# hzxie/RMNet

Measured on AMD Instinct MI355X. Metric: frames/sec at 480p, 1 object, T=5 memory; memory-read HBM GB/s vs peak, higher is better.
Workload: dtype f32 convs; memory read = fp16 operands (K, V, q, P rounded to 11 bits), fp32 accumulate (RMNET_BANK_F16): the frame loop's default for clips with one object -- on one-object 480x854 clips whose masks HAVE a boundary (tests/live_fixture.py) mask IoU vs the CPU path 0.99993-0.99997 and foreground logi

## Files before the change

### include/rmnet_hip.h

```cpp
#ifndef RMNET_HIP_H_
#define RMNET_HIP_H_

#include <stddef.h>
#include <stdint.h>

#ifdef __cplusplus
extern "C" {
#endif

#define RMNET_ABI_VERSION 6

enum {
  RMNET_OK = 0,
  RMNET_E_INVALID_ARG = -1,
  RMNET_E_WORKSPACE = -2,
  RMNET_E_LAUNCH = -3,
  RMNET_E_UNSUPPORTED = -4
};

int rmnet_abi_version(void);
const char *rmnet_error_string(int code);

size_t rmnet_region_map_workspace_bytes(int B, int K, int H, int W);
int rmnet_region_map_f32(const float *mask, int B, int K, int H, int W, float prob_threshold,
                         int n_pts_threshold, int n_bbox_loose_pixels, float *att_map,
                         int32_t *bboxes, int32_t *cell_rects, int pad_l, int pad_t,
                         int cell_stride, int cells_h, int cells_w, void *workspace,
                         size_t workspace_bytes, void *stream);

int rmnet_region_map_warped_f32(const float *mask, const float *flow, int B, int K, int H, int W,
                                float prob_threshold, int n_pts_threshold, int n_bbox_loose_pixels,
                                float *att_map, int32_t *bboxes, int32_t *cell_rects, int pad_l,
                                int pad_t, int cell_stride, int cells_h, int cells_w, float *warped,
                                void *workspace, size_t workspace_bytes, void *stream);

int rmnet_boxes_to_cell_rects_i32(const int32_t *bboxes, int n_boxes, int k_per_batch, int pad_l,
                                  int pad_t, int cell_stride, int cells_h, int cells_w,
                                  int32_t *cell_rects, void *stream);

#define RMNET_MR_DEFAULT 0
#define RMNET_MR_FORCE_GENERIC 1
#define RMNET_MR_EXACT_FP32 2
#define RMNET_MR_F16 4
#define RMNET_BANK_F16 4
#define RMNET_MR_QX 8
#define RMNET_BANK_QX 8

size_t rmnet_memory_read_workspace_bytes(int no, int De, int Do, int T, int h, int w, int flags);
int rmnet_memory_read_f32(const float *m_key, const float *m_val, const float *q_key,
                          const float *q_val, int no, int De, int Do, int T, int h, int w,
                          long long m_chan_stride, long long m_obj_stride, long long v_chan_stride,
                          long long v_obj_stride, float *mem_val, float *p_out,
                          const int32_t *mem_rects, const int32_t *qry_rects, int flags,
                          void *workspace, size_t workspace_bytes, void *stream);

int rmnet_memory_read_f32_ev(const float *m_key, const float *m_val, const float *q_key,
                             const float *q_val, int no, int De, int Do, int T, int h, int w,
                             long long m_chan_stride, long long m_obj_stride,
                             long long v_chan_stride, long long v_obj_stride, float *mem_val,
                             float *p_out, const int32_t *mem_rects, const int32_t *qry_rects,
                             int flags, void *workspace, size_t workspace_bytes, void *stream,
                             void *ev_start, void *ev_mid, void *ev_end);

size_t rmnet_bank_bytes(int no, int Tcap, int h, int w);
size_t rmnet_bank_overflow_offset(int no, int Tcap, int h, int w);
size_t rmnet_bank_area_offset(int no, int Tcap, int h, int w);
int rmnet_bank_append_f32(void *bank, int no, int Tcap, int h, int w, int slot, const float *k4,
                          const float *v4, const int32_t *rects, void *stream);
int rmnet_bank_append_f32_at(void *bank, int no, int Tcap, int h, int w, int slot, const int32_t *slot_dev,
                             const float *k4, const float *v4, const int32_t *rects, void *stream);
int rmnet_bank_read_f32_at(void *bank, int no, int Tcap, int h, int w, int T, const int32_t *T_dev, int flags,
                           const float *q_key, const float *q_val, const int32_t *qry_rects,
                           float *mem_val, void *workspace, size_t workspace_bytes, void *stream,
                           void *ev_start, void *ev_mid, void *ev_end);
size_t rmnet_bank_read_workspace_bytes(int no, int h, int w);
size_t rmnet_bank_read_workspace_bytes_for(int no, int h, int w, int T);
int rmnet_bank_read_f32(void *bank, int no, int Tcap, int h, int w, int T,
                        const float *q_key, const float *q_val, const int32_t *qry_rects,
                        float *mem_val, void *workspace, size_t workspace_bytes, void *stream,
                        void *ev_start, void *ev_mid, void *ev_end);

int rmnet_rect_mask_f32(const float *x, int n, int C, int T, int h, int w, const int32_t *rects,
                        float *y, void *stream);

int rmnet_channel_affine_f32(const float *x, const float *scale, const float *shift,
                             const float *res, const float *res_scale, const float *res_shift,
                             int relu, long long N, int C, long long HW, float *out, void *stream);

int rmnet_affine_relu_maxpool_f32(const float *x, const float *scale, const float *shift, long long N,
                                  int C, int H, int W, float *out, void *stream);

int rmnet_upsample2x_add_f32(const float *x, const float *skip, long long N, int C, int h, int w,
                             float *out, void *stream);

int rmnet_channel_affine_nhwc_f32(const float *x, const float *scale, const float *shift, const float *res, const float *res_scale,
                                  const float *res_shift, int relu, long long rows, int C, float *out, void *stream);
int rmnet_upsample2x_add_nhwc_f32(const float *x, const float *skip, long long N, int C, int h, int w, float *out, void *stream);
int rmnet_affine_relu_maxpool_nhwc_f32(const float *x, const float *scale, const float *shift, long long N, int C, int H, int W,
                                       float *out, void *stream);

#define RMNET_CONV_RELU_IN 1
#define RMNET_CONV_RELU_OUT 2
int rmnet_conv3x3_split_f32(const float *x, const void *wpack, const float *w_unscale, const float *bias, const float *res, int flags,
                            int N, int H, int W, int Cin, float *out, int32_t *range_word, void *stream);

int rmnet_conv3x3_split_lds_f32(const float *x, const void *wpack, const float *w_unscale, const float *bias, const float *res,
                                int flags, int N, int H, int W, int Cin, float *out, int32_t *range_word, void *stream);

int rmnet_conv3x3_rows_f32(const float *x, const void *wpack, const float *w_unscale, const float *bias, const float *res, int flags,
                           int N, int H, int W, int Cin, float *out, int32_t *range_word, void *stream);

int rmnet_conv_split_f32(const float *x, const void *wpack, const float *w_unscale, const float *shift, const float *res, int flags,
                         int N, int H, int W, int Cin, int Cout, int ksize, int stride, float *out, float *out2, int out_split,
                         int32_t *range_word, void *stream);

#define RMNET_CONV_X_SPLIT 4
#define RMNET_CONV_OUT_SPLIT 8
int rmnet_conv_split_pre_f32(const void *x, const void *wpack, const float *w_unscale, const float *shift, const float *res, int flags,
                             int N, int H, int W, int Cin, int Cout, int ksize, int stride, void *out, float *out2, int out_split,
                             int32_t *range_word, void *stream);
int rmnet_split_act_f32(const float *x, long long M, int C, int relu, void *out, int32_t *range_word, void *stream);

int rmnet_stem_split_f32(const float *frame, const float *mask, const float *other, const void *wpack, const float *w_unscale,
                         const float *shift, int N, int H, int W, float *out, int32_t *range_word, void *stream);

int rmnet_pred_head_f32(const float *x, const float *w, const float *bias, int n, int Hq, int Wq, int C, float *out, void *stream);

#define RMNET_FLOW_RELU 1
#define RMNET_FLOW_LEAKY 2
#define RMNET_FLOW_TRANSPOSED 4
int rmnet_flow_conv_f32(const float *x, int x_ld, const void *wpack, const float *w_unscale, const float *shift, int flags, int N, int H,
                        int W, int Cin, int Cout, int ksize, int stride, float *out, int out_ld, int coff, int32_t *range_word,
                        void *stream);

size_t rmnet_flow_head_workspace_bytes(int N, int H, int W, int Cin);
int rmnet_flow_head_f32(const float *x, int x_ld, const float *wpack, const float *bias, int N, int H, int W, int Cin, float *out,
                        void *workspace, size_t workspace_bytes, void *stream);

int rmnet_flow_up_f32(const float *flow, const float *w, int N, int h, int w_, float *out, int out_ld, int coff, void *stream);

int rmnet_soft_aggregate_f32(const float *dec, const int32_t *obj_begin, int B, int K, int Hp, int Wp,
                             int pad_l, int pad_t, int H, int W, float *logit, float *prob,
                             void *stream);

int rmnet_flow_affine_f32(const float *flow, const float *m1, const float *m2, int H, int W,
                          float *out, void *stream);
size_t rmnet_flow_affine_workspace_bytes(int H, int W);
int rmnet_flow_affine_f32_host(const float *flow_host, const float *m1_host, const float *m2_host,
                               int H, int W, float *out_host, void *workspace,
                               size_t workspace_bytes, void *stream);

#ifdef __cplusplus
}
#endif
#endif
```

### rmnet_amd/_lib.py

```python

import ctypes
import os

_HERE = os.path.dirname(os.path.abspath(__file__))
LIB_PATH = os.environ.get('RMNET_HIP_LIB') or os.path.join(_HERE, 'librmnet_hip.so')

c_f32p = ctypes.c_void_p
c_i32p = ctypes.c_void_p

SIGNATURES = {
    'rmnet_abi_version': (ctypes.c_int, []),
    'rmnet_error_string': (ctypes.c_char_p, [ctypes.c_int]),
    'rmnet_region_map_workspace_bytes': (ctypes.c_size_t, [ctypes.c_int] * 4),
    'rmnet_region_map_f32': (ctypes.c_int, [
        c_f32p, ctypes.c_int, ctypes.c_int, ctypes.c_int, ctypes.c_int, ctypes.c_float, ctypes.c_int,
        ctypes.c_int, c_f32p, c_i32p, c_i32p, ctypes.c_int, ctypes.c_int, ctypes.c_int, ctypes.c_int,
        ctypes.c_int, ctypes.c_void_p, ctypes.c_size_t, ctypes.c_void_p]),
    'rmnet_region_map_warped_f32': (ctypes.c_int, [
        c_f32p, c_f32p, ctypes.c_int, ctypes.c_int, ctypes.c_int, ctypes.c_int, ctypes.c_float, ctypes.c_int,
        ctypes.c_int, c_f32p, c_i32p, c_i32p, ctypes.c_int, ctypes.c_int, ctypes.c_int, ctypes.c_int,
        ctypes.c_int, c_f32p, ctypes.c_void_p, ctypes.c_size_t, ctypes.c_void_p]),
    'rmnet_boxes_to_cell_rects_i32': (ctypes.c_int, [
        c_i32p, ctypes.c_int, ctypes.c_int, ctypes.c_int, ctypes.c_int, ctypes.c_int, ctypes.c_int,
        ctypes.c_int, c_i32p, ctypes.c_void_p]),
    'rmnet_memory_read_workspace_bytes': (ctypes.c_size_t, [ctypes.c_int] * 7),
    'rmnet_memory_read_f32': (ctypes.c_int, [
        c_f32p, c_f32p, c_f32p, c_f32p, ctypes.c_int, ctypes.c_int, ctypes.c_int, ctypes.c_int,
        ctypes.c_int, ctypes.c_int, ctypes.c_longlong, ctypes.c_longlong, ctypes.c_longlong,
        ctypes.c_longlong, c_f32p, c_f32p, c_i32p, c_i32p, ctypes.c_int, ctypes.c_void_p,
        ctypes.c_size_t, ctypes.c_void_p]),
    'rmnet_memory_read_f32_ev': (ctypes.c_int, [
        c_f32p, c_f32p, c_f32p, c_f32p, ctypes.c_int, ctypes.c_int, ctypes.c_int, ctypes.c_int,
        ctypes.c_int, ctypes.c_int, ctypes.c_longlong, ctypes.c_longlong, ctypes.c_longlong,
        ctypes.c_longlong, c_f32p, c_f32p, c_i32p, c_i32p, ctypes.c_int, ctypes.c_void_p,
        ctypes.c_size_t, ctypes.c_void_p, ctypes.c_void_p, ctypes.c_void_p, ctypes.c_void_p]),
    'rmnet_bank_bytes': (ctypes.c_size_t, [ctypes.c_int] * 4),
    'rmnet_bank_overflow_offset': (ctypes.c_size_t, [ctypes.c_int] * 4),
    'rmnet_bank_area_offset': (ctypes.c_size_t, [ctypes.c_int] * 4),
    'rmnet_bank_append_f32': (ctypes.c_int, [
        ctypes.c_void_p, ctypes.c_int, ctypes.c_int, ctypes.c_int, ctypes.c_int, ctypes.c_int, c_f32p,
        c_f32p, c_i32p, ctypes.c_void_p]),
    'rmnet_bank_append_f32_at': (ctypes.c_int, [
        ctypes.c_void_p, ctypes.c_int, ctypes.c_int, ctypes.c_int, ctypes.c_int, ctypes.c_int, c_i32p, c_f32p,
        c_f32p, c_i32p, ctypes.c_void_p]),
    'rmnet_bank_read_f32_at': (ctypes.c_int, [
        ctypes.c_void_p, ctypes.c_int, ctypes.c_int, ctypes.c_int, ctypes.c_int, ctypes.c_int, c_i32p, ctypes.c_int, c_f32p,
        c_f32p, c_i32p, c_f32p, ctypes.c_void_p, ctypes.c_size_t, ctypes.c_void_p, ctypes.c_void_p,
        ctypes.c_void_p, ctypes.c_void_p]),
    'rmnet_bank_read_workspace_bytes': (ctypes.c_size_t, [ctypes.c_int] * 3),
    'rmnet_bank_read_workspace_bytes_for': (ctypes.c_size_t, [ctypes.c_int] * 4),
    'rmnet_bank_read_f32': (ctypes.c_int, [
        ctypes.c_void_p, ctypes.c_int, ctypes.c_int, ctypes.c_int, ctypes.c_int, ctypes.c_int, c_f32p,
        c_f32p, c_i32p, c_f32p, ctypes.c_void_p, ctypes.c_size_t, ctypes.c_void_p, ctypes.c_void_p,
        ctypes.c_void_p, ctypes.c_void_p]),
    'rmnet_rect_mask_f32': (ctypes.c_int, [
        c_f32p, ctypes.c_int, ctypes.c_int, ctypes.c_int, ctypes.c_int, ctypes.c_int, c_i32p, c_f32p,
        ctypes.c_void_p]),
    'rmnet_channel_affine_f32': (ctypes.c_int, [
        c_f32p, c_f32p, c_f32p, c_f32p, c_f32p, c_f32p, ctypes.c_int, ctypes.c_longlong, ctypes.c_int,
        ctypes.c_longlong, c_f32p, ctypes.c_void_p]),
    'rmnet_upsample2x_add_f32': (ctypes.c_int, [
        c_f32p, c_f32p, ctypes.c_longlong, ctypes.c_int, ctypes.c_int, ctypes.c_int, c_f32p, ctypes.c_void_p]),
    'rmnet_soft_aggregate_f32': (ctypes.c_int, [
        c_f32p, c_i32p, ctypes.c_int, ctypes.c_int, ctypes.c_int, ctypes.c_int, ctypes.c_int, ctypes.c_int,
        ctypes.c_int, ctypes.c_int, c_f32p, c_f32p, ctypes.c_void_p]),
    'rmnet_affine_relu_maxpool_f32': (ctypes.c_int, [
        c_f32p, c_f32p, c_f32p, ctypes.c_longlong, ctypes.c_int, ctypes.c_int, ctypes.c_int, c_f32p,
        ctypes.c_void_p]),
    'rmnet_channel_affine_nhwc_f32': (ctypes.c_int, [
        c_f32p, c_f32p, c_f32p, c_f32p, c_f32p, c_f32p, ctypes.c_int, ctypes.c_longlong, ctypes.c_int, c_f32p, ctypes.c_void_p]),
    'rmnet_upsample2x_add_nhwc_f32': (ctypes.c_int, [
        c_f32p, c_f32p, ctypes.c_longlong, ctypes.c_int, ctypes.c_int, ctypes.c_int, c_f32p, ctypes.c_void_p]),
    'rmnet_affine_relu_maxpool_nhwc_f32': (ctypes.c_int, [
        c_f32p, c_f32p, c_f32p, ctypes.c_longlong, ctypes.c_int, ctypes.c_int, ctypes.c_int, c_f32p, ctypes.c_void_p]),
    'rmnet_conv3x3_split_f32': (ctypes.c_int, [
        c_f32p, ctypes.c_void_p, c_f32p, c_f32p, c_f32p, ctypes.c_int, ctypes.c_int, ctypes.c_int, ctypes.c_int, ctypes.c_int,
        c_f32p, c_i32p, ctypes.c_void_p]),
    'rmnet_conv3x3_split_lds_f32': (ctypes.c_int, [
        c_f32p, ctypes.c_void_p, c_f32p, c_f32p, c_f32p, ctypes.c_int, ctypes.c_int, ctypes.c_int, ctypes.c_int, ctypes.c_int,
        c_f32p, c_i32p, ctypes.c_void_p]),
    'rmnet_conv3x3_rows_f32': (ctypes.c_int, [
        c_f32p, ctypes.c_void_p, c_f32p, c_f32p, c_f32p, ctypes.c_int, ctypes.c_int, ctypes.c_int, ctypes.c_int, ctypes.c_int,
        c_f32p, c_i32p, ctypes.c_void_p]),
    'rmnet_conv_split_f32': (ctypes.c_int, [
        c_f32p, ctypes.c_void_p, c_f32p, c_f32p, c_f32p, ctypes.c_int, ctypes.c_int, ctypes.c_int, ctypes.c_int, ctypes.c_int,
        ctypes.c_int, ctypes.c_int, ctypes.c_int, c_f32p, c_f32p, ctypes.c_int, c_i32p, ctypes.c_void_p]),
    'rmnet_conv_split_pre_f32': (ctypes.c_int, [
        ctypes.c_void_p, ctypes.c_void_p, c_f32p, c_f32p, c_f32p, ctypes.c_int, ctypes.c_int, ctypes.c_int, ctypes.c_int, ctypes.c_int,
        ctypes.c_int, ctypes.c_int, ctypes.c_int, ctypes.c_void_p, c_f32p, ctypes.c_int, c_i32p, ctypes.c_void_p]),
    'rmnet_split_act_f32': (ctypes.c_int, [
        c_f32p, ctypes.c_longlong, ctypes.c_int, ctypes.c_int, ctypes.c_void_p, c_i32p, ctypes.c_void_p]),
    'rmnet_stem_split_f32': (ctypes.c_int, [
        c_f32p, c_f32p, c_f32p, ctypes.c_void_p, c_f32p, c_f32p, ctypes.c_int, ctypes.c_int, ctypes.c_int, c_f32p, c_i32p,
        ctypes.c_void_p]),
    'rmnet_pred_head_f32': (ctypes.c_int, [
        c_f32p, c_f32p, c_f32p, ctypes.c_int, ctypes.c_int, ctypes.c_int, ctypes.c_int, c_f32p, ctypes.c_void_p]),
    'rmnet_flow_conv_f32': (ctypes.c_int, [
        c_f32p, ctypes.c_int, ctypes.c_void_p, c_f32p, c_f32p, ctypes.c_int, ctypes.c_int, ctypes.c_int, ctypes.c_int, ctypes.c_int,
        ctypes.c_int, ctypes.c_int, ctypes.c_int, c_f32p, ctypes.c_int, ctypes.c_int, c_i32p, ctypes.c_void_p]),
    'rmnet_flow_head_workspace_bytes': (ctypes.c_size_t, [ctypes.c_int] * 4),
    'rmnet_flow_head_f32': (ctypes.c_int, [
        c_f32p, ctypes.c_int, c_f32p, c_f32p, ctypes.c_int, ctypes.c_int, ctypes.c_int, ctypes.c_int, c_f32p, ctypes.c_void_p,
        ctypes.c_size_t, ctypes.c_void_p]),
    'rmnet_flow_up_f32': (ctypes.c_int, [
        c_f32p, c_f32p, ctypes.c_int, ctypes.c_int, ctypes.c_int, c_f32p, ctypes.c_int, ctypes.c_int, ctypes.c_void_p]),
    'rmnet_flow_affine_f32': (ctypes.c_int, [
        c_f32p, c_f32p, c_f32p, ctypes.c_int, ctypes.c_int, c_f32p, ctypes.c_void_p]),
    'rmnet_flow_affine_workspace_bytes': (ctypes.c_size_t, [ctypes.c_int, ctypes.c_int]),
    'rmnet_flow_affine_f32_host': (ctypes.c_int, [
        ctypes.c_void_p, ctypes.c_void_p, ctypes.c_void_p, ctypes.c_int, ctypes.c_int,
        ctypes.c_void_p, ctypes.c_void_p, ctypes.c_size_t, ctypes.c_void_p]),
}

ABI_VERSION = 6
_lib = None


class RMNetHipError(RuntimeError):
    pass


def load():
    global _lib
    if _lib is not None:
        return _lib
    if not os.path.exists(LIB_PATH):
        raise RMNetHipError(
            'librmnet_hip.so is missing (%s). The HIP kernels are the only implementation of this '
            'path; build them with `python -m rmnet_amd.build`.' % LIB_PATH)
    lib = ctypes.CDLL(LIB_PATH)
    for name, (res, args) in SIGNATURES.items():
        fn = getattr(lib, name)
        fn.restype = res
        fn.argtypes = args
    if lib.rmnet_abi_version() != ABI_VERSION:
        raise RMNetHipError('librmnet_hip.so ABI %d != expected %d' % (lib.rmnet_abi_version(), ABI_VERSION))
    _lib = lib
    return lib


def check(code, what):
    if code != 0:
        msg = load().rmnet_error_string(code).decode()
        raise RMNetHipError('%s failed: %s (code %d)' % (what, msg, code))
```

### rmnet_amd/build.py

```python

import os
import shutil
import subprocess

HERE = os.path.dirname(os.path.abspath(__file__))
CSRC = os.path.join(HERE, 'csrc')
SOURCES = ['capi.hip', 'region_map.hip', 'flow_affine.hip', 'memory_read.hip', 'bank.hip', 'epilogue.hip', 'conv3x3.hip', 'conv3x3_rows.hip', 'conv_split.hip',
           'stem.hip', 'pred_head.hip', 'flow_conv.hip', 'flow_head.hip']
LIB = os.path.join(HERE, 'librmnet_hip.so')
ARCH = 'gfx950'


def hipcc_path():
    for cand in (shutil.which('hipcc'), '/opt/rocm/bin/hipcc'):
        if cand and os.path.exists(cand):
            return cand
    raise RuntimeError('hipcc not found: librmnet_hip.so cannot be built')


def needs_build():
    if not os.path.exists(LIB):
        return True
    t = os.path.getmtime(LIB)
    deps = [os.path.join(CSRC, s) for s in SOURCES] + [
        os.path.join(CSRC, 'common.h'),
        os.path.join(os.path.dirname(HERE), 'include', 'rmnet_hip.h')]
    return any(os.path.getmtime(d) > t for d in deps)


def build_library(force=False, verbose=False):
    if not force and not needs_build():
        return LIB
    cmd = [hipcc_path(), '--offload-arch=' + ARCH, '-O3', '-std=c++17', '-shared', '-fPIC',
           '-o', LIB] + [os.path.join(CSRC, s) for s in SOURCES]
    if verbose:
        print(' '.join(cmd))
    subprocess.check_call(cmd, cwd=CSRC)
    return LIB


if __name__ == '__main__':
    print(build_library(force=True, verbose=True))
```

### rmnet_amd/ops.py

```python

import ctypes
import os

import numpy as np
import torch

from . import _lib


MR_FORCE_GENERIC = 1
MR_EXACT_FP32 = 2
BANK_MAX_SLOTS = 2048


def _check(t, name, dtype=torch.float32):
    if not isinstance(t, torch.Tensor):
        raise RuntimeError('%s must be a torch.Tensor' % name)
    if not t.is_cuda:
        raise RuntimeError('%s must be a CUDA tensor' % name)
    if not t.is_contiguous():
        raise RuntimeError('%s must be contiguous' % name)
    if t.dtype != dtype:
        raise RuntimeError('%s must be %s, got %s' % (name, dtype, t.dtype))

# ... 447 lines not shown
    amax = w.abs().amax(dim=(1, 2, 3))
    _, ex = torch.frexp(amax)
    e = torch.where(amax > 0, 15 - ex, torch.zeros_like(ex))
    ws = torch.ldexp(w, e.view(-1, 1, 1, 1).to(w.dtype))
    hi = ws.half()
    lo = (ws - hi.float()).half()
    planes = torch.stack([p.reshape(CONV_COUT, cin // 32, 32, 9).permute(3, 1, 0, 2) for p in (hi, lo)], dim=2)
    unscale = torch.ldexp(torch.ones_like(amax), (-e).to(amax.dtype))
    return planes.contiguous().view(-1).view(torch.int16), unscale.contiguous()


_range_words = {}


def conv_range_word(device):
    idx = torch.device(device).index
    idx = torch.cuda.current_device() if idx is None else idx
    w = _range_words.get(idx)
    if w is None:
        w = _range_words[idx] = torch.zeros(1, dtype=torch.int32, device=torch.device('cuda', idx))
    return w


CONV3X3_KERNEL_DEFAULT = 'wreg'
CONV3X3_ENTRIES = {'wreg': 'rmnet_conv3x3_split_f32', 'lds': 'rmnet_conv3x3_split_lds_f32'}


def conv3x3_entry():
    v = os.environ.get('RMNET_CONV3X3_KERNEL')
    v = CONV3X3_KERNEL_DEFAULT if v is None else v.strip()
    if v not in CONV3X3_ENTRIES:
        raise RuntimeError('RMNET_CONV3X3_KERNEL must be one of %s, got %r' % (sorted(CONV3X3_ENTRIES), v))
    return CONV3X3_ENTRIES[v]


CONV3X3_ROWS_DEFAULT = True
CONV3X3_ROWS_ENTRY = 'rmnet_conv3x3_rows_f32'
CONV3X3_ROWS_CIN = 256


def conv3x3_rows_enabled():
    v = os.environ.get('RMNET_CONV3X3_ROWS')
    if v is None:
        return CONV3X3_ROWS_DEFAULT
    if v.strip() not in ('0', '1'):
        raise RuntimeError("RMNET_CONV3X3_ROWS must be '0' or '1', got %r" % v)
    return v.strip() == '1'


def conv3x3_split(x, wpack, w_unscale, bias=None, res=None, relu_in=False, relu_out=False, out=None, range_word=None):
    _check_act(x, 'x')
    if x.dim() != 4 or not x.is_contiguous(memory_format=torch.channels_last):
        raise RuntimeError('x must be a channels-last [N, Cin, H, W] tensor')
    N, cin, H, W = x.shape
    if cin % 32:
        raise RuntimeError('conv3x3_split needs Cin % 32 == 0, got %d' % cin)
    _check(wpack, 'wpack', torch.int16)
    if wpack.numel() != 9 * cin * CONV_COUT * 2:
        raise RuntimeError('wpack has %d elements, a Cin = %d pack has %d' % (wpack.numel(), cin, 9 * cin * CONV_COUT * 2))
    _check(w_unscale, 'w_unscale')
    shape = (N, CONV_COUT, H, W)
    for t, n in ((bias, 'bias'),):
        if t is not None:
            _check(t, n)
            if t.numel() != CONV_COUT:
                raise RuntimeError('%s must have 256 elements' % n)
    if w_unscale.numel() != CONV_COUT:
        raise RuntimeError('w_unscale must have 256 elements')
    if res is not None:
        _check_act(res, 'res')
        if tuple(res.shape) != shape or not res.is_contiguous(memory_format=torch.channels_last):
            raise RuntimeError('res must be a channels-last [N, 256, H, W] tensor')
    if out is None:
        out = torch.empty(shape, dtype=x.dtype, device=x.device, memory_format=torch.channels_last)
    else:
        _check_act(out, 'out')
        if tuple(out.shape) != shape or not out.is_contiguous(memory_format=torch.channels_last):
            raise RuntimeError('out must be a channels-last [N, 256, H, W] tensor')
    if range_word is not None:
        _check(range_word, 'range_word', torch.int32)
    for t in (wpack, w_unscale, bias, res, out, range_word):
        if t is not None and t.device != x.device:
            raise RuntimeError('conv3x3_split: every tensor must be on %s' % x.device)
    flags = (CONV_RELU_IN if relu_in else 0) | (CONV_RELU_OUT if relu_out else 0)
    entry = conv3x3_entry()
    if conv3x3_rows_enabled() and os.environ.get('RMNET_CONV3X3_KERNEL') is None and cin == CONV3X3_ROWS_CIN:
        entry = CONV3X3_ROWS_ENTRY
    lib = _lib.load()
    with torch.cuda.device(x.device):
        rc = getattr(lib, entry)(_ptr(x), _ptr(wpack), _ptr(w_unscale), _ptr(bias), _ptr(res), flags, N, H, W, cin,
                                 _ptr(out), _ptr(range_word), _stream(x.device))
    _lib.check(rc, entry)
    return out


@torch.no_grad()
def conv_split_pack(weight, bn_scale=None):
    if weight.dim() != 4 or weight.shape[2] != weight.shape[3] or weight.shape[2] not in (1, 3) or weight.shape[1] % 32 \
            or weight.shape[0] % 64:
        raise RuntimeError('conv_split_pack needs a [Cout, Cin, k, k] weight with k in (1, 3), Cin % 32 == 0 and Cout % 64 == 0, '
                           'got %s' % (tuple(weight.shape),))
    if weight.dtype != torch.float32:
        raise RuntimeError('conv_split_pack needs fp32 weights, got %s' % weight.dtype)
    cout, cin, k = weight.shape[0], weight.shape[1], weight.shape[2]
    w = weight.detach().double()
    if bn_scale is not None:
        if bn_scale.numel() != cout:
            raise RuntimeError('bn_scale must have Cout = %d elements' % cout)
        w = w * bn_scale.detach().to(w.device, torch.float64).view(-1, 1, 1, 1)
    amax = w.abs().amax(dim=(1, 2, 3))
    _, ex = torch.frexp(amax)
    e = torch.where(amax > 0, 15 - ex, torch.zeros_like(ex))
    ws = torch.ldexp(w, e.view(-1, 1, 1, 1).to(w.dtype))
    hi = ws.half()
    lo = (ws - hi.double()).half()
    planes = torch.stack([p.reshape(cout, cin // 32, 32, k * k).permute(3, 1, 0, 2) for p in (hi, lo)], dim=2)
    unscale = torch.ldexp(torch.ones_like(amax), (-e).to(amax.dtype)).float()
    return planes.contiguous().view(-1).view(torch.int16), unscale.contiguous()


CONV_X_SPLIT, CONV_OUT_SPLIT = 4, 8


def is_split_act(t):
    return isinstance(t, torch.Tensor) and t.dtype == torch.float16 and t.dim() == 6 and tuple(t.shape[4:]) == (2, 32)


def _check_split_act(t, name):
    if not is_split_act(t):
        raise RuntimeError('%s must be a split activation: torch.float16 [N, H, W, C // 32, 2, 32]' % name)
    if not t.is_cuda:
        raise RuntimeError('%s must be a CUDA tensor' % name)
    if not t.is_contiguous():
        raise RuntimeError('%s must be contiguous' % name)


def split_act(x, relu=False, range_word=None):
    _check_act(x, 'x')
    if x.dim() != 4 or not x.is_contiguous(memory_format=torch.channels_last):
        raise RuntimeError('x must be a channels-last [N, C, H, W] tensor')
    N, C, H, W = x.shape
    if C % 32 or x.numel() == 0:
        raise RuntimeError('split_act needs C % 32 == 0 and a non-empty tensor, got %s' % (tuple(x.shape),))
    if range_word is not None:
        _check(range_word, 'range_word', torch.int32)
        if range_word.device != x.device:
            raise RuntimeError('split_act: every tensor must be on %s' % x.device)
    out = torch.empty((N, H, W, C // 32, 2, 32), dtype=torch.float16, device=x.device)
    lib = _lib.load()
    with torch.cuda.device(x.device):
        rc = lib.rmnet_split_act_f32(_ptr(x), N * H * W, C, 1 if relu else 0, _ptr(out), _ptr(range_word), _stream(x.device))
    _lib.check(rc, 'rmnet_split_act_f32')
    return out


def conv_split(x, wpack, w_unscale, shift=None, res=None, ksize=3, stride=1, relu_in=False, relu_out=False, out=None,
               range_word=None, split=None, out_presplit=False):
    x_split = is_split_act(x)
    if x_split:
        _check_split_act(x, 'x')
        N, H, W = x.shape[:3]
        cin = x.shape[3] * 32
        if relu_in:
            raise RuntimeError('conv_split: relu_in cannot be applied to a split activation (its producer applies it)')
    else:
        _check_act(x, 'x')
        if x.dim() != 4 or not x.is_contiguous(memory_format=torch.channels_last):
            raise RuntimeError('x must be a channels-last [N, Cin, H, W] tensor')
        N, cin, H, W = x.shape
    if ksize not in (1, 3) or stride not in (1, 2):
        raise RuntimeError('conv_split implements ksize 1 / 3 and stride 1 / 2, got %r / %r' % (ksize, stride))
    _check(w_unscale, 'w_unscale')
    cout = w_unscale.numel()
    if cin % 32 or cout % 64 or cout == 0:
        raise RuntimeError('conv_split needs Cin % 32 == 0 and Cout % 64 == 0, got %d, %d' % (cin, cout))
    _check(wpack, 'wpack', torch.int16)
    if wpack.numel() != ksize * ksize * cin * cout * 2:
        raise RuntimeError('wpack has %d elements, a %dx%d Cin = %d Cout = %d pack has %d'
                           % (wpack.numel(), ksize, ksize, cin, cout, ksize * ksize * cin * cout * 2))
    pad = ksize // 2
    shape = (N, cout, (H + 2 * pad - ksize) // stride + 1, (W + 2 * pad - ksize) // stride + 1)
    if shift is not None:
        _check(shift, 'shift')
        if shift.numel() != cout:
            raise RuntimeError('shift must have Cout = %d elements' % cout)
    if res is not None:
        _check_act(res, 'res')
        if tuple(res.shape) != shape or not res.is_contiguous(memory_format=torch.channels_last):
            raise RuntimeError('res must be a channels-last %s tensor' % (shape,))
    out2 = None
    if out_presplit:
        if split is not None or out is not None:
            raise RuntimeError('conv_split: out_presplit returns one new split activation, without split / out')
        out = torch.empty((N, shape[2], shape[3], cout // 32, 2, 32), dtype=torch.float16, device=x.device)
    elif split is not None:
        if res is not None or out is not None or not 0 < split < cout or split % 4:
            raise RuntimeError('conv_split: split must be a multiple of 4 in (0, %d), without res / out' % cout)
        out = torch.empty((N, split) + shape[2:], dtype=torch.float32, device=x.device, memory_format=torch.channels_last)
        out2 = torch.empty((N, cout - split) + shape[2:], dtype=torch.float32, device=x.device, memory_format=torch.channels_last)
    elif out is None:
        out = torch.empty(shape, dtype=torch.float32, device=x.device, memory_format=torch.channels_last)
    else:
        _check_act(out, 'out')
        if tuple(out.shape) != shape or not out.is_contiguous(memory_format=torch.channels_last):
            raise RuntimeError('out must be a channels-last %s tensor' % (shape,))
    if range_word is not None:
        _check(range_word, 'range_word', torch.int32)
    for t in (wpack, w_unscale, shift, res, out, range_word):
        if t is not None and t.device != x.device:
            raise RuntimeError('conv_split: every tensor must be on %s' % x.device)
    flags = (CONV_RELU_IN if relu_in else 0) | (CONV_RELU_OUT if relu_out else 0)
    lib = _lib.load()
    with torch.cuda.device(x.device):
        if x_split or out_presplit:
            flags |= (CONV_X_SPLIT if x_split else 0) | (CONV_OUT_SPLIT if out_presplit else 0)
            what = 'rmnet_conv_split_pre_f32'
            rc = lib.rmnet_conv_split_pre_f32(_ptr(x), _ptr(wpack), _ptr(w_unscale), _ptr(shift), _ptr(res), flags, N, H, W, cin,
                                              cout, ksize, stride, _ptr(out), _ptr(out2), split or 0, _ptr(range_word),
                                              _stream(x.device))
        else:
            what = 'rmnet_conv_split_f32'
            rc = lib.rmnet_conv_split_f32(_ptr(x), _ptr(wpack), _ptr(w_unscale), _ptr(shift), _ptr(res), flags, N, H, W, cin, cout,
                                          ksize, stride, _ptr(out), _ptr(out2), split or 0, _ptr(range_word), _stream(x.device))
    _lib.check(rc, what)
    return out if out2 is None else (out, out2)


FLOW_RELU, FLOW_LEAKY, FLOW_TRANSPOSED = 1, 2, 4
_FLOW_ACT = {None: 0, False: 0, 'none': 0, True: FLOW_RELU, 'relu': FLOW_RELU, 'leaky': FLOW_LEAKY}


def flow_conv_phase_weights(weight):
    w = weight.permute(1, 0, 2, 3)
    phases = []
    for a in (0, 1):
        for b in (0, 1):
            ky = torch.tensor([3 - a, 1 - a], device=w.device)
            kx = torch.tensor([3 - b, 1 - b], device=w.device)
            phases.append(w.index_select(2, ky).index_select(3, kx))
    return torch.stack(phases, 0)


@torch.no_grad()
def flow_conv_pack(weight, transposed=False):
    if weight.dim() != 4 or weight.shape[2] != weight.shape[3] or weight.shape[2] not in ((4,) if transposed else (3, 5)):
        raise RuntimeError('flow_conv_pack needs a [Cout, Cin, k, k] weight with k in (3, 5), or transposed a [Cin, Cout, 4, 4] one, '
                           'got %s' % (tuple(weight.shape),))
    if weight.dtype != torch.float32:
        raise RuntimeError('flow_conv_pack needs fp32 weights, got %s' % weight.dtype)
    w = weight.detach().double()
    w = flow_conv_phase_weights(w) if transposed else w.unsqueeze(0)
    P, cout, cin, kh, kw = w.shape
    if cout % 64:
        raise RuntimeError('flow_conv_pack needs Cout % 64 == 0, got ' + str(cout))
    cp = (cin + 31) // 32 * 32
    amax = w.abs().amax(dim=(0, 2, 3, 4))
    _, ex = torch.frexp(amax)
    e = torch.where(amax > 0, 15 - ex, torch.zeros_like(ex))
    ws = torch.ldexp(w, e.view(1, -1, 1, 1, 1).to(w.dtype))
    hi = ws.half()
    lo = (ws - hi.double()).half()
    pad = lambda p: torch.nn.functional.pad(p, (0, 0, 0, 0, 0, cp - cin))
    planes = torch.stack([pad(p).reshape(P, cout, cp // 32, 32, kh * kw).permute(0, 4, 2, 1, 3) for p in (hi, lo)], dim=3)
    unscale = torch.ldexp(torch.ones_like(amax), (-e).to(amax.dtype)).float()
    return planes.contiguous().view(-1).view(torch.int16), unscale.contiguous()


def flow_conv_out_hw(H, W, ksize, stride, transposed):
    if transposed:
        return 2 * H, 2 * W
    pad = ksize // 2
    return (H + 2 * pad - ksize) // stride + 1, (W + 2 * pad - ksize) // stride + 1


def flow_conv(x, wpack, w_unscale, shift=None, *, ksize=3, stride=1, transposed=False, act=None, cin=None, out=None, out_coff=0,
              range_word=None):
    _check_act(x, 'x')
    if x.dim() != 4 or not x.is_contiguous(memory_format=torch.channels_last):
        raise RuntimeError('x must be a channels-last [N, C, H, W] tensor')
    if transposed:
        if ksize != 4 or stride != 2:
            raise RuntimeError('flow_conv implements the transposed convolution for ksize 4 / stride 2, got %r / %r' % (ksize, stride))
    elif ksize not in (3, 5) or stride not in (1, 2):
        raise RuntimeError('flow_conv implements ksize 3 / 5 and stride 1 / 2, got %r / %r' % (ksize, stride))
    if act not in _FLOW_ACT:
        raise RuntimeError("act must be None, 'relu' or 'leaky', got %r" % (act,))
    N, x_ld, H, W = x.shape
    cin = x_ld if cin is None else int(cin)
    cp = (cin + 31) // 32 * 32
    if cin <= 0 or x_ld % 4 or x_ld < cp:
        raise RuntimeError('flow_conv needs x_ld %% 4 == 0 and x_ld >= ceil32(cin): x has %d channels for cin = %d' % (x_ld, cin))
    _check(w_unscale, 'w_unscale')
    cout = w_unscale.numel()
    if cout % 64 or cout == 0:
        raise RuntimeError('flow_conv needs Cout % 64 == 0, got ' + str(cout))
    _check(wpack, 'wpack', torch.int16)
    want = (16 if transposed else ksize * ksize) * cp * cout * 2
    if wpack.numel() != want:
        raise RuntimeError('wpack has %d elements, a %dx%d%s cin = %d Cout = %d pack has %d'
                           % (wpack.numel(), ksize, ksize, ' transposed' if transposed else '', cin, cout, want))
    if shift is not None:
        _check(shift, 'shift')
        if shift.numel() != cout:
            raise RuntimeError('shift must have Cout = %d elements' % cout)
    Ho, Wo = flow_conv_out_hw(H, W, ksize, stride, transposed)
    if out is None:
        if out_coff:
            raise RuntimeError('out_coff without out')
        out = torch.empty((N, cout, Ho, Wo), dtype=x.dtype, device=x.device, memory_format=torch.channels_last)
    else:
        _check_act(out, 'out')
        if out.dim() != 4 or not out.is_contiguous(memory_format=torch.channels_last) or \
                (out.shape[0], out.shape[2], out.shape[3]) != (N, Ho, Wo):
            raise RuntimeError('out must be a channels-last [%d, out_ld, %d, %d] tensor' % (N, Ho, Wo))
        if out.shape[1] % 4 or out_coff % 4 or out_coff < 0 or out_coff + cout > out.shape[1]:
            raise RuntimeError('flow_conv needs out_ld %% 4 == 0, out_coff %% 4 == 0 and out_coff + Cout <= out_ld, got %d, %d, %d'
                               % (out.shape[1], out_coff, cout))
    if range_word is not None:
        _check(range_word, 'range_word', torch.int32)
    for t in (wpack, w_unscale, shift, out, range_word):
        if t is not None and t.device != x.device:
            raise RuntimeError('flow_conv: every tensor must be on %s' % x.device)
    flags = _FLOW_ACT[act] | (FLOW_TRANSPOSED if transposed else 0)
    lib = _lib.load()
    with torch.cuda.device(x.device):
        rc = lib.rmnet_flow_conv_f32(_ptr(x), x_ld, _ptr(wpack), _ptr(w_unscale), _ptr(shift), flags, N, H, W, cin, cout, ksize, stride,
                                     _ptr(out), out.shape[1], out_coff, _ptr(range_word), _stream(x.device))
    _lib.check(rc, 'rmnet_flow_conv_f32')
    return out


FLOW_HEAD_SLICE = 32


@torch.no_grad()
def flow_head_pack(weight):
    if not isinstance(weight, torch.Tensor) or weight.dim() != 4 or weight.shape[0] != 2 or tuple(weight.shape[2:]) != (3, 3) \
            or weight.shape[1] < 1:
        raise RuntimeError('flow_head_pack needs a [2, Cin, 3, 3] weight, got %s' % (tuple(getattr(weight, 'shape', ())),))
    if weight.dtype != torch.float32:
        raise RuntimeError('flow_head_pack needs fp32 weights, got %s' % weight.dtype)
    cin = weight.shape[1]
    cp = (cin + FLOW_HEAD_SLICE - 1) // FLOW_HEAD_SLICE * FLOW_HEAD_SLICE
    pack = torch.zeros(cp, 9, 2, dtype=torch.float32, device=weight.device)
    pack[:cin] = weight.detach().permute(1, 2, 3, 0).reshape(cin, 9, 2)
    return pack.view(-1)


def flow_head(x, wpack, bias, cin=None):
    _check_act(x, 'x')
    if x.dim() != 4 or not x.is_contiguous(memory_format=torch.channels_last):
        raise RuntimeError('x must be a channels-last [N, C, H, W] tensor')
    N, x_ld, H, W = x.shape
    cin = x_ld if cin is None else int(cin)
    if cin <= 0 or x_ld % 4 or x_ld < cin:
        raise RuntimeError('flow_head needs x_ld %% 4 == 0 and x_ld >= cin >= 1: x has %d channels for cin = %d' % (x_ld, cin))
    _check(wpack, 'wpack')
    want = (cin + FLOW_HEAD_SLICE - 1) // FLOW_HEAD_SLICE * FLOW_HEAD_SLICE * 18
    if wpack.numel() != want:
        raise RuntimeError('wpack has %d elements, a cin = %d flow-head pack has %d' % (wpack.numel(), cin, want))
    _check(bias, 'bias')
    if bias.numel() != 2:
        raise RuntimeError('bias must have 2 elements')
    if wpack.device != x.device or bias.device != x.device:
        raise RuntimeError('flow_head: every tensor must be on %s' % x.device)
    if N == 0 or H == 0 or W == 0:
        raise RuntimeError('flow_head needs a non-empty x, got %s' % (tuple(x.shape),))
    out = torch.empty((N, 2, H, W), dtype=x.dtype, device=x.device)
    lib = _lib.load()
    with torch.cuda.device(x.device):
        nb = lib.rmnet_flow_head_workspace_bytes(N, H, W, cin)
        ws = _ws(nb, x.device)
# ... 184 lines not shown
```

Before: 631.2.

## Add row-staged LDS 3x3 conv kernel for split-precision trunk convolutions

Adds a new conv_rows kernel for same-channel 3x3 stride-1 convs on split fp16 hi/lo activations. Each block stages a contiguous run of pixel rows, plus halo rows, into LDS once per kernel row. It reuses that staging across the three horizontal taps, with masked lanes pointed at zero rows. The kernel uses MFMA with a weight prefetch pipeline and explicit scheduling barriers, and is routed by default for 128 and 256 channel trunk convs. It aims to cut redundant global reads and staging compared with the existing split conv path, at the cost of large LDS use (about 134 KB) and therefore low occupancy.

```diff
diff --git a/include/rmnet_hip.h b/include/rmnet_hip.h
--- a/include/rmnet_hip.h
+++ b/include/rmnet_hip.h
@@ -121,6 +121,10 @@
                              int32_t *range_word, void *stream);
 int rmnet_split_act_f32(const float *x, long long M, int C, int relu, void *out, int32_t *range_word, void *stream);
 
+int rmnet_conv_rows_pre_f32(const void *x, const void *wpack, const float *w_unscale, const float *shift, const float *res, int flags,
+                            int N, int H, int W, int Cin, int Cout, int ksize, int stride, void *out, float *out2, int out_split,
+                            int32_t *range_word, void *stream);
+
 int rmnet_stem_split_f32(const float *frame, const float *mask, const float *other, const void *wpack, const float *w_unscale,
                          const float *shift, int N, int H, int W, float *out, int32_t *range_word, void *stream);
 
diff --git a/rmnet_amd/_lib.py b/rmnet_amd/_lib.py
--- a/rmnet_amd/_lib.py
+++ b/rmnet_amd/_lib.py
@@ -88,6 +88,9 @@
     'rmnet_conv_split_pre_f32': (ctypes.c_int, [
         ctypes.c_void_p, ctypes.c_void_p, c_f32p, c_f32p, c_f32p, ctypes.c_int, ctypes.c_int, ctypes.c_int, ctypes.c_int, ctypes.c_int,
         ctypes.c_int, ctypes.c_int, ctypes.c_int, ctypes.c_void_p, c_f32p, ctypes.c_int, c_i32p, ctypes.c_void_p]),
+    'rmnet_conv_rows_pre_f32': (ctypes.c_int, [
+        ctypes.c_void_p, ctypes.c_void_p, c_f32p, c_f32p, c_f32p, ctypes.c_int, ctypes.c_int, ctypes.c_int, ctypes.c_int, ctypes.c_int,
+        ctypes.c_int, ctypes.c_int, ctypes.c_int, ctypes.c_void_p, c_f32p, ctypes.c_int, c_i32p, ctypes.c_void_p]),
     'rmnet_split_act_f32': (ctypes.c_int, [
         c_f32p, ctypes.c_longlong, ctypes.c_int, ctypes.c_int, ctypes.c_void_p, c_i32p, ctypes.c_void_p]),
     'rmnet_stem_split_f32': (ctypes.c_int, [
diff --git a/rmnet_amd/build.py b/rmnet_amd/build.py
--- a/rmnet_amd/build.py
+++ b/rmnet_amd/build.py
@@ -6,7 +6,7 @@
 HERE = os.path.dirname(os.path.abspath(__file__))
 CSRC = os.path.join(HERE, 'csrc')
 SOURCES = ['capi.hip', 'region_map.hip', 'flow_affine.hip', 'memory_read.hip', 'bank.hip', 'epilogue.hip', 'conv3x3.hip', 'conv3x3_rows.hip', 'conv_split.hip',
-           'stem.hip', 'pred_head.hip', 'flow_conv.hip', 'flow_head.hip']
+           'conv_rows.hip', 'stem.hip', 'pred_head.hip', 'flow_conv.hip', 'flow_head.hip']
 LIB = os.path.join(HERE, 'librmnet_hip.so')
 ARCH = 'gfx950'
 
diff --git a/rmnet_amd/csrc/conv_rows.hip b/rmnet_amd/csrc/conv_rows.hip
--- /dev/null
+++ b/rmnet_amd/csrc/conv_rows.hip
@@ -0,0 +1,296 @@
+#include <mutex>
+
+#include "common.h"
+
+namespace rmnet {
+namespace {
+
+typedef _Float16 half8 __attribute__((ext_vector_type(8)));
+typedef _Float16 half4 __attribute__((ext_vector_type(4)));
+typedef float f32x4 __attribute__((ext_vector_type(4)));
+typedef unsigned int u32x4 __attribute__((ext_vector_type(4)));
+
+constexpr int kKT = 32;
+constexpr int kThreads = 512;
+constexpr float kActScale = 64.0f;
+constexpr float kActUnscale = 1.0f / 64.0f;
+constexpr float kF16Max = 65504.0f;
+constexpr int kTileElems = 32768;
+constexpr int kZeroRows = 4;
+constexpr int kAhead = 1;
+constexpr int kStageBatch = 8;
+constexpr int kStagePasses = 16;
+
+constexpr int rows_mt(int C) { return kTileElems / C; }
+constexpr int rows_lds_bytes(int C) { return (rows_mt(C) + 2 + kZeroRows) * C * 4; }
+static_assert(rows_lds_bytes(256) == 137216 && rows_lds_bytes(128) == 134144 && rows_lds_bytes(64) == 132608, "(MT + 6) rows x C x 4 B");
+static_assert(rows_lds_bytes(256) <= kLdsBytesPerCU, "LDS budget");
+
+__device__ inline int swzr(int row, int chunk) { return row * kKT + ((chunk ^ ((row >> 1) & 2)) << 3); }
+
+__device__ inline void split4(const f32x4 v, half4& hi, half4& lo, int& bad) {
+#pragma unroll
+  for (int e = 0; e < 4; ++e) {
+    const float y = v[e] * kActScale;
+    bad += !(fabsf(y) <= kF16Max) ? 1 : 0;
+    const float c = fminf(fmaxf(y, -kF16Max), kF16Max);
+    const _Float16 h = (_Float16)c;
+    hi[e] = h;
+    lo[e] = (_Float16)(c - (float)h);
+  }
+}
+
+struct RowsArgs {
+  const _Float16* xs;
+  const half8* wp;
+  const float* unscale;
+  const float* shift;
+  float* out;
+  _Float16* outs;
+  int* range;
+  int M, H, W, relu_out;
+};
+
+extern __shared__ __attribute__((aligned(16))) _Float16 conv_rows_lds[];
+
+template <int C, bool OS>
+__global__ __launch_bounds__(kThreads) void conv_rows(RowsArgs a) {
+  constexpr int MT = rows_mt(C);
+  constexpr int CB = C / kKT;
+  constexpr int kStaged = MT + 2;
+  constexpr int kPlaneHalves = (kStaged + kZeroRows) * kKT;
+  constexpr int kBlockHalves = 2 * kPlaneHalves;
+  constexpr int kWPlane = C * kKT;
+  constexpr int kPassRows = 2 * (kThreads / 16) / CB;
+  static_assert(C % kKT == 0 && CB % 2 == 0 && MT % 128 == 0 && (MT / 128) * CB == 8, "8 waves of 128 pixels x 32 channels");
+  static_assert(kStaged % 4 == 2, "the zero row of a masked lane: (kStaged + (row + 2) % 4) % 4 == row % 4");
+  static_assert(kPassRows % 8 == 0 && kPassRows * kStagePasses == MT, "a pass keeps the swizzle bit; 16 passes stage MT rows");
+  static_assert(kStagePasses % kStageBatch == 0, "whole batches");
+  _Float16* const lds = conv_rows_lds;
+  const int tid = threadIdx.x, lane = tid & 63, wave = tid >> 6;
+  const int wc = wave % CB, wp = wave / CB;
+  const int fr = lane & 15, fc = lane >> 4;
+  const int m0 = blockIdx.x * MT;
+  const int HW = a.H * a.W;
+
+  if (tid < 16 * 2 * CB) *reinterpret_cast<half8*>(lds + (tid >> 4) * kPlaneHalves + kStaged * kKT + 8 * (tid & 15)) = half8{0, 0, 0, 0, 0, 0, 0, 0};
+
+  unsigned inside[3] = {0u, 0u, 0u};
+#pragma unroll
+  for (int i = 0; i < 8; ++i) {
+    const int m = m0 + 128 * wp + 16 * i + fr;
+    const bool pin = m < a.M;
+    const int r = (pin ? m : 0) % HW;
+    const int ph = r / a.W, pw = r % a.W;
+    unsigned bits = 0;
+#pragma unroll
+    for (int t = 0; t < 9; ++t) {
+      const int h = ph + t / 3 - 1, w = pw + t % 3 - 1;
+      bits |= (pin && h >= 0 && h < a.H && w >= 0 && w < a.W ? 1u : 0u) << t;
+    }
+    inside[i / 3] |= bits << (9 * (i % 3));
+  }
+
+  const int sch = tid & 3, spl = (tid >> 3) & 1, sblk = (tid >> 4) % CB;
+  const int srow = 2 * ((tid >> 4) / CB) + ((tid >> 2) & 1);
+  const unsigned scol = sblk * (2 * kKT) + spl * kKT + 8 * sch;
+  _Float16* const sdst = lds + sblk * kBlockHalves + spl * kPlaneHalves + swzr(srow, sch);
+  auto stage = [&](int ty) __attribute__((always_inline)) {
+    int qb = m0 + (ty - 1) * a.W - 1;
+    asm volatile("" : "+s"(qb));
+    auto src = [&](int row) {
+      const int q = min(max(qb + row, 0), a.M - 1);
+      return reinterpret_cast<const u32x4*>(a.xs + ((unsigned)q * (unsigned)(2 * C) + scol));
+    };
+#pragma unroll
+    for (int g = 0; g < kStagePasses / kStageBatch; ++g) {
+      u32x4 v[kStageBatch];
+#pragma unroll
+      for (int k = 0; k < kStageBatch; ++k) v[k] = *src(srow + kPassRows * (kStageBatch * g + k));
+#pragma unroll
+      for (int k = 0; k < kStageBatch; ++k) *reinterpret_cast<u32x4*>(sdst + kPassRows * (kStageBatch * g + k) * kKT) = v[k];
+    }
+    if (tid < 16 * CB) {
+      const u32x4 v = *src(srow + MT);
+      *reinterpret_cast<u32x4*>(sdst + MT * kKT) = v;
+    }
+  };
+
+  half8 wa[4], wb[4];
+  const half8* wsrc = a.wp;
+  const half8* const wlast = a.wp + (9 * CB - 1) * (2 * kWPlane / 8);
+  const unsigned wl = (wc * 32 + fr) * 4 + fc;
+  auto load_w = [&](half8(&w)[4]) __attribute__((always_inline)) {
+#pragma unroll
+    for (int j = 0; j < 2; ++j)
+#pragma unroll
+      for (int p = 0; p < 2; ++p) w[2 * j + p] = wsrc[wl + (unsigned)(p * (kWPlane / 8) + j * 64)];
+    wsrc = wsrc == wlast ? wsrc : wsrc + 2 * kWPlane / 8;
+  };
+
+  f32x4 acc[8][2], accx[8][2];
+#pragma unroll
+  for (int i = 0; i < 8; ++i)
+#pragma unroll
+    for (int j = 0; j < 2; ++j) acc[i][j] = accx[i][j] = f32x4{0.f, 0.f, 0.f, 0.f};
+
+  auto run_tap = [&](int tap) __attribute__((always_inline)) {
+    const int dx1 = tap % 3;
+    unsigned ao[8];
+#pragma unroll
+    for (int i = 0; i < 8; ++i) {
+      const bool in = (inside[i / 3] >> (9 * (i % 3) + tap)) & 1;
+      const int row = 128 * wp + 16 * i + fr + dx1;
+      const unsigned real = (unsigned)swzr(row, fc);
+      ao[i] = in ? real : (unsigned)((kStaged + ((row + 2) & 3)) * kKT) + (real & (kKT - 1));
+    }
+    half8 bh[kAhead + 1], bl[kAhead + 1];
+    auto frag = [&](int n) __attribute__((always_inline)) {
+      const _Float16* p = lds + ao[n & 7] + (n >> 3) * kBlockHalves;
+      bh[n % (kAhead + 1)] = *reinterpret_cast<const half8*>(p);
+      bl[n % (kAhead + 1)] = *reinterpret_cast<const half8*>(p + kPlaneHalves);
+    };
+    auto mma = [&](int cb, const half8(&w)[4]) __attribute__((always_inline)) {
+#pragma unroll
+      for (int i = 0; i < 8; ++i) {
+        if (8 * cb + i + kAhead < 8 * CB) frag(8 * cb + i + kAhead);
+        const half8 h = bh[(8 * cb + i) % (kAhead + 1)], l = bl[(8 * cb + i) % (kAhead + 1)];
+#pragma unroll
+        for (int j = 0; j < 2; ++j) acc[i][j] = __builtin_amdgcn_mfma_f32_16x16x32_f16(w[2 * j], h, acc[i][j], 0, 0, 0);
+#pragma unroll
+        for (int j = 0; j < 2; ++j) accx[i][j] = __builtin_amdgcn_mfma_f32_16x16x32_f16(w[2 * j], l, accx[i][j], 0, 0, 0);
+#pragma unroll
+        for (int j = 0; j < 2; ++j) accx[i][j] = __builtin_amdgcn_mfma_f32_16x16x32_f16(w[2 * j + 1], h, accx[i][j], 0, 0, 0);
+      }
+    };
+    auto step = [&](int cb, const half8(&wcur)[4], half8(&wnxt)[4]) __attribute__((always_inline)) {
+      __builtin_amdgcn_sched_barrier(0);
+      load_w(wnxt);
+      __builtin_amdgcn_sched_barrier(0);
+      mma(cb, wcur);
+#pragma unroll
+      for (int i = 0; i < 8; ++i) {
+        __builtin_amdgcn_sched_group_barrier(0x100, 2, 0);
+        __builtin_amdgcn_sched_group_barrier(0x008, 6, 0);
+      }
+    };
+#pragma unroll
+    for (int n = 0; n < kAhead; ++n) frag(n);
+#pragma unroll
+    for (int cb = 0; cb < CB; cb += 2) {
+      step(cb, wa, wb);
+      step(cb + 1, wb, wa);
+    }
+    __builtin_amdgcn_sched_barrier(0);
+  };
+
+  load_w(wa);
+#pragma unroll 1
+  for (int ty = 0; ty < 3; ++ty) {
+    __syncthreads();
+    stage(ty);
+    __syncthreads();
+#pragma unroll 1
+    for (int tx = 0; tx < 3; ++tx) run_tap(3 * ty + tx);
+  }
+
+  int me = m0 + 128 * wp;
+  asm volatile("" : "+v"(me));
+  int bad = 0;
+#pragma unroll
+  for (int j = 0; j < 2; ++j) {
+    const int co = wc * 32 + j * 16 + 4 * fc;
+    const f32x4 us = *reinterpret_cast<const f32x4*>(a.unscale + co) * kActUnscale;
+    const f32x4 b = a.shift ? *reinterpret_cast<const f32x4*>(a.shift + co) : f32x4{0.f, 0.f, 0.f, 0.f};
+#pragma unroll
+    for (int i = 0; i < 8; ++i) acc[i][j] = (acc[i][j] + accx[i][j]) * us + b;
+  }
+#pragma unroll
+  for (int j = 0; j < 2; ++j)
+#pragma unroll
+    for (int i = 0; i < 8; ++i) asm volatile("" : "+v"(acc[i][j]));
+#pragma unroll
+  for (int j = 0; j < 2; ++j) {
+    const int co = wc * 32 + j * 16 + 4 * fc;
+#pragma unroll
+    for (int i = 0; i < 8; ++i) {
+      const int m = me + i * 16 + fr;
+      if (m >= a.M) continue;
+      f32x4 v = acc[i][j];
+      if (a.relu_out) {
+#pragma unroll
+        for (int e = 0; e < 4; ++e) v[e] = v[e] < 0.0f ? 0.0f : v[e];
+      }
+      if constexpr (OS) {
+        half4 hi, lo;
+        split4(v, hi, lo, bad);
+        _Float16* o = a.outs + (size_t)m * (2 * C) + (co >> 5) * (2 * kKT) + (co & 31);
+        *reinterpret_cast<half4*>(o) = hi;
+        *reinterpret_cast<half4*>(o + kKT) = lo;
+      } else {
+        *reinterpret_cast<f32x4*>(a.out + (size_t)m * C + co) = v;
+      }
+    }
+  }
+  if (a.range && bad) atomicAdd(a.range, bad);
+}
+
+template <int C, bool OS>
+int rows_launch(const RowsArgs& a, hipStream_t st) {
+  static std::mutex mu;
+  static bool done[64] = {};
+  int dev = 0;
+  if (hipGetDevice(&dev) != hipSuccess || dev < 0 || dev >= 64) return RMNET_E_LAUNCH;
+  {
+    std::lock_guard<std::mutex> lock(mu);
+    if (!done[dev]) {
+      hipStreamCaptureStatus cs = hipStreamCaptureStatusNone;
+      if (hipStreamIsCapturing(st, &cs) != hipSuccess) return RMNET_E_LAUNCH;
+      if (cs != hipStreamCaptureStatusNone) return RMNET_E_UNSUPPORTED;
+      if (hipFuncSetAttribute(reinterpret_cast<const void*>(conv_rows<C, OS>), hipFuncAttributeMaxDynamicSharedMemorySize,
+                              rows_lds_bytes(C)) != hipSuccess)
+        return RMNET_E_LAUNCH;
+      done[dev] = true;
+    }
+  }
+  hipLaunchKernelGGL((conv_rows<C, OS>), dim3((unsigned)((a.M + rows_mt(C) - 1) / rows_mt(C))), dim3(kThreads), rows_lds_bytes(C), st, a);
+  return check_launch();
+}
+
+inline bool overlap(const void* p, long long pn, const void* q, long long qn) {
+  const char* a = reinterpret_cast<const char*>(p);
+  const char* b = reinterpret_cast<const char*>(q);
+  return a < b + qn && b < a + pn;
+}
+
+}
+}
+
+extern "C" int rmnet_conv_rows_pre_f32(const void* x, const void* wpack, const float* w_unscale, const float* shift, const float* res,
+                                       int flags, int N, int H, int W, int Cin, int Cout, int ksize, int stride, void* out, float* out2,
+                                       int out_split, int32_t* range_word, void* stream) {
+  using namespace rmnet;
+  if (flags & ~(RMNET_CONV_RELU_IN | RMNET_CONV_RELU_OUT | RMNET_CONV_X_SPLIT | RMNET_CONV_OUT_SPLIT)) return RMNET_E_INVALID_ARG;
+  const bool xs = (flags & RMNET_CONV_X_SPLIT) != 0, os = (flags & RMNET_CONV_OUT_SPLIT) != 0;
+  if (!x || !wpack || !w_unscale || !out || N <= 0 || H <= 0 || W <= 0 || Cin <= 0 || Cout <= 0) return RMNET_E_INVALID_ARG;
+  if (xs && (flags & RMNET_CONV_RELU_IN)) return RMNET_E_INVALID_ARG;
+  if (os && out2) return RMNET_E_INVALID_ARG;
+  if ((reinterpret_cast<uintptr_t>(x) | reinterpret_cast<uintptr_t>(wpack) | reinterpret_cast<uintptr_t>(w_unscale) |
+       reinterpret_cast<uintptr_t>(shift) | reinterpret_cast<uintptr_t>(res) | reinterpret_cast<uintptr_t>(out) |
+       reinterpret_cast<uintptr_t>(out2)) & 15)
+    return RMNET_E_INVALID_ARG;
+  if (out2 && (res || out_split <= 0 || out_split >= Cout || out_split % 4)) return RMNET_E_INVALID_ARG;
+  if (!xs || ksize != 3 || stride != 1 || Cin != Cout || (Cin != 64 && Cin != 128 && Cin != 256) || res || out2) return RMNET_E_UNSUPPORTED;
+  const long long M = (long long)N * H * W;
+  if (M * Cin >= (1LL << 31)) return RMNET_E_UNSUPPORTED;
+  if (overlap(out, M * Cout * 4, x, M * Cin * 4)) return RMNET_E_INVALID_ARG;
+  RowsArgs a;
+  a.xs = reinterpret_cast<const _Float16*>(x); a.wp = reinterpret_cast<const half8*>(wpack); a.unscale = w_unscale; a.shift = shift;
+  a.out = os ? nullptr : reinterpret_cast<float*>(out); a.outs = os ? reinterpret_cast<_Float16*>(out) : nullptr;
+  a.range = range_word; a.M = (int)M; a.H = H; a.W = W;
+  a.relu_out = (flags & RMNET_CONV_RELU_OUT) != 0;
+  hipStream_t st = (hipStream_t)stream;
+  if (Cin == 256) return os ? rows_launch<256, true>(a, st) : rows_launch<256, false>(a, st);
+  if (Cin == 128) return os ? rows_launch<128, true>(a, st) : rows_launch<128, false>(a, st);
+  return os ? rows_launch<64, true>(a, st) : rows_launch<64, false>(a, st);
+}
diff --git a/rmnet_amd/ops.py b/rmnet_amd/ops.py
--- a/rmnet_amd/ops.py
+++ b/rmnet_amd/ops.py
@@ -623,6 +623,21 @@
         rc = lib.rmnet_split_act_f32(_ptr(x), N * H * W, C, 1 if relu else 0, _ptr(out), _ptr(range_word), _stream(x.device))
     _lib.check(rc, 'rmnet_split_act_f32')
     return out
+
+
+TRUNK_ROWS_DEFAULT = True
+TRUNK_ROWS_ENTRY = 'rmnet_conv_rows_pre_f32'
+TRUNK_ROWS_ALL = (64, 128, 256)
+TRUNK_ROWS_CLASSES = (128, 256)
+
+
+def trunk_rows_enabled():
+    v = os.environ.get('RMNET_TRUNK_ROWS')
+    if v is None:
+        return TRUNK_ROWS_DEFAULT
+    if v.strip() not in ('0', '1'):
+        raise RuntimeError("RMNET_TRUNK_ROWS must be '0' or '1', got %r" % v)
+    return v.strip() == '1'
 
 
 def conv_split(x, wpack, w_unscale, shift=None, res=None, ksize=3, stride=1, relu_in=False, relu_out=False, out=None,
@@ -681,14 +696,16 @@
         if t is not None and t.device != x.device:
             raise RuntimeError('conv_split: every tensor must be on %s' % x.device)
     flags = (CONV_RELU_IN if relu_in else 0) | (CONV_RELU_OUT if relu_out else 0)
+    rows = trunk_rows_enabled() and x_split and ksize == 3 and stride == 1 and cin == cout and cin in TRUNK_ROWS_CLASSES \
+        and res is None and split is None
     lib = _lib.load()
     with torch.cuda.device(x.device):
         if x_split or out_presplit:
             flags |= (CONV_X_SPLIT if x_split else 0) | (CONV_OUT_SPLIT if out_presplit else 0)
-            what = 'rmnet_conv_split_pre_f32'
-            rc = lib.rmnet_conv_split_pre_f32(_ptr(x), _ptr(wpack), _ptr(w_unscale), _ptr(shift), _ptr(res), flags, N, H, W, cin,
-                                              cout, ksize, stride, _ptr(out), _ptr(out2), split or 0, _ptr(range_word),
-                                              _stream(x.device))
+            what = TRUNK_ROWS_ENTRY if rows else 'rmnet_conv_split_pre_f32'
+            rc = getattr(lib, what)(_ptr(x), _ptr(wpack), _ptr(w_unscale), _ptr(shift), _ptr(res), flags, N, H, W, cin,
+                                    cout, ksize, stride, _ptr(out), _ptr(out2), split or 0, _ptr(range_word),
+                                    _stream(x.device))
         else:
             what = 'rmnet_conv_split_f32'
             rc = lib.rmnet_conv_split_f32(_ptr(x), _ptr(wpack), _ptr(w_unscale), _ptr(shift), _ptr(res), flags, N, H, W, cin, cout,
```

Result: faster. 640.7, median of 6 (+1.5%).
